# ppwwyyxx/speaker-recognition

Measured on AMD Instinct MI355X. Metric: frames/sec scored (MFCC+GMM), higher is better.
Workload: dtype f32

## Files before the change

speaker-recognition_amd/csrc/abi_options.cpp:

```cpp
#include "abi_internal.hpp"

#include "bw_plan.hpp"
#include "bw_stats.hpp"
#include "calib.hpp"
#include "calib_plan.hpp"
#include "diar.hpp"
#include "diar_plan.hpp"
#include "em.hpp"
#include "featnorm.hpp"
#include "featnorm_plan.hpp"
#include "fork_proxy.hpp"
#include "gmm_full.hpp"
#include "jfa.hpp"
#include "jfa_plan.hpp"
#include "kmeans_init.hpp"
#include "map_batch.hpp"
#include "map_plan.hpp"
#include "mfcc.hpp"
#include "norm_plan.hpp"
#include "plda.hpp"
#include "plda_plan.hpp"
#include "score.hpp"
#include "score_norm.hpp"
#include "silence.hpp"
// ... 18 lines not shown
    const std::string k(key);
    if (k == "score_frames_per_lane") {
        if (value != 0 && value != 1 && value != 2 && value != 4) fail("frames per lane must be 0/1/2/4");
        score_options().frames_per_lane = (int)value;
    } else if (k == "score_model_groups") {
        score_options().model_groups = (int)value;
    } else if (k == "score_packed") {
        score_options().packed = (int)value;
    } else if (k == "score_engine") {
        if (value < 0 || value > 6 || value == 2)
            fail("score_engine must be 0 (auto), 1 (vector ALU), 3 (split-bf16 matrix cores), 4 (split-bf16, shared-sigma form), "
                 "5 (split-fp16 matrix cores) or 6 (split-fp16, shared-sigma form); 2 was the fp32 matrix-core engine, removed in round 5 "
                 "(never selected: 1.45-1.8x slower than split-bf16 at the same accuracy)");
        score_options().engine = (int)value;
    } else if (k == "score_h2s_shape") {
        if (value < 0 || value > 6)
            fail("score_h2s_shape must be 0 (automatic), 1 (4-wave workgroups), 2 (12-wave workgroups), 3 (12 waves, image loop pipelined inside the wave), "
                 "4 (4 waves on one tile, the block's models split between them), 5 (as 3, on the flat image where 3 takes the compact one) "
                 "or 6 (as 3, one quadratic half per block where 3 forms one per two blocks)");
        score_options().h2s_shape = (int)value;
    } else if (k == "flush_list_cap") {
        if (value < 0) fail("flush_list_cap must be >= 0");
        score_options().flush_list_cap = (int)value;
    } else if (k == "score_h2s_pack_tails") {
        if (value != 0 && value != 1) fail("score_h2s_pack_tails must be 0 or 1");
        score_options().h2s_pack_tails = (int)value;
    } else if (k == "score_h2s_force_exc") {
        score_options().h2s_force_exc = value != 0;
    } else if (k == "score_split_shape") {
        if (value != 0 && value != 1 && value != 8 && value != 12 && value != 16)
            fail("score_split_shape must be 0 (automatic), 1 (4-wave workgroups) or 8 / 12 / 16 (waves of the wide, pipelined form)");
        score_options().split_shape = (int)value;
    } else if (k == "score_mfma_ft") {
        if (value < 0 || value > 4) fail("score_mfma_ft must be 0..4");
// ... 92 lines not shown
```

speaker-recognition_amd/csrc/gmm_model.cpp:

```cpp
#include "gmm_model.hpp"
#include "score_shapes.hpp"

#include <atomic>
#include <algorithm>
#include <cmath>
#include <limits>
#include <cstdlib>
#include <cstring>
#include <thread>

namespace sr {
uint64_t next_gmm_uid() {
    static std::atomic<uint64_t> next{1};
    return next.fetch_add(1);
}
}

namespace sr {

namespace {

template <class F>
void host_parallel_for(int n, size_t cost_per_piece, F work) {
    const size_t total = (size_t)n * cost_per_piece;
// ... 746 lines not shown
            }
        }
        amp_t[thr] = amp_l;
        coef_t[thr] = coef_l;
    });
    for (int t = 0; t < MAX_T; t++) {
        pm.amp = std::max(pm.amp, amp_t[t]);
        pm.coef_max = std::max(pm.coef_max, coef_t[t]);
    }
    pm.pad_waste = 1.0 - ((double)K * S) / ((double)pm.n_tiles * MT * n_blocks * SHARED_SB);
    pm.ref = pack_models_split({models[0]}, SPLIT_F16X2);
    return pm;
}

PackedH2Compact pack_h2_compact(const PackedH2Shared &pm, int dim) {
    PackedH2Compact pc;
    if (pm.params.empty() || !h2c_applies(dim, pm.klf)) return pc;
    const int h = h2c_half_steps(dim);
    const H2cMap m = h2c_map(h);
    pc.nk = m.nk;
    pc.nf = m.nf;
    pc.nb = m.nb;
    const int c_slot = 8 * h - 1;
    auto flat_slot = [&](bool linear, int part, int s) {
        if (s < dim) return part == 1 ? s : linear ? 2 * dim + 1 + s : 2 * dim + s;
        if (linear && s == c_slot) return part == 1 ? dim : 3 * dim + 1;
        return -1;
    };
    auto b_desc = [&](bool linear, int part, int s) -> uint16_t {
        if (s < dim) return (uint16_t)(s | ((part == 1 ? 1 : 2) << 8));
        if (linear && s == c_slot && part == 1) return (uint16_t)(3 << 8);
        return 0;
    };
    pc.q_desc.assign((size_t)m.nb * 16, 0);
// ... 98 lines not shown
```

speaker-recognition_amd/csrc/gmm_model.hpp:

```cpp
#pragma once

#include "common.hpp"

#include <memory>
#include <string>
#include <vector>

struct SRModelSet;

namespace sr {
uint64_t next_gmm_uid();
}

struct GMM {
    int nr_mixtures = 0;
    int covariance_type = 1;
    int dim = 0;
    std::vector<double> weights;
    std::vector<double> mean;
    std::vector<double> sigma;
    mutable std::shared_ptr<SRModelSet> single[sr::MAX_DEVICES];
    uint64_t uid = sr::next_gmm_uid();
    uint64_t generation = 0;
    void drop_single() {
// ... 78 lines not shown
    std::vector<uint16_t> params;
    std::vector<SharedBlock> blocks;
    std::vector<float> center, scale;
    std::vector<uint16_t> q_desc, l_desc;
    double amp = 0.0, pad_waste = 0.0, sigma_ratio = 1.0, coef_max = 0.0;
    PackedSplit ref;
};
PackedH2Shared pack_models_h2_shared(const std::vector<const GMM *> &models);
struct PackedH2Compact {
    int nk = 0, nf = 0, nb = 0;
    std::vector<uint16_t> params;
    std::vector<SharedBlock> blocks;
    std::vector<uint16_t> q_desc, l_desc;
};
PackedH2Compact pack_h2_compact(const PackedH2Shared &pm, int dim);
struct WorkItem { int t[4]; };
std::vector<WorkItem> pack_tail_tiles(const std::vector<int> &counts, int frames_per_tile, bool pack_tails);
void mel_sweep_starts(const int *col0, const int *cnt, int n_bands, const int pass_len[4], int *start);
int mel_sweep_extra_cycles(const int *start, const int *cnt, int n_bands, int pass);
bool models_share_sigma_and_weights(const std::vector<const GMM *> &models);
PackedBx3Shared pack_models_bx3_shared(const std::vector<const GMM *> &models);
void split_bf16x3(float v, uint16_t out[3]);
void split_f16x2(float v, uint16_t out[2]);
uint16_t f32_to_f16_rne(float v);
float f16_to_f32(uint16_t h);

}

struct SRModelSet {
    sr::PackedModels host;
// ... 7 lines not shown
    bool bx3_stale = false;
    sr::PackedSplit h2;
    sr::DevBuf<uint16_t> d_h2_params;
    sr::DevBuf<float> d_h2_center, d_h2_scale;
    sr::DevBuf<sr::ChunkDesc> d_h2_chunks;
    sr::PackedBx3Shared shared;
    sr::DevBuf<uint16_t> d_shared_params;
    sr::DevBuf<sr::SharedBlock> d_shared_blocks;
    sr::DevBuf<float> d_shared_center;
    sr::PackedH2Shared h2s;
    sr::DevBuf<uint16_t> d_h2s_params, d_h2s_qdesc, d_h2s_ldesc, d_h2s_ref_params;
    sr::DevBuf<sr::SharedBlock> d_h2s_blocks;
    sr::DevBuf<float> d_h2s_center, d_h2s_scale, d_h2s_ref_center, d_h2s_ref_scale;
    sr::DevBuf<sr::ChunkDesc> d_h2s_ref_chunks;
    sr::DevBuf<int> d_h2s_ref_gcb;
    int h2c_state = 0;
    int h2c_nk = 0;
    sr::DevBuf<uint16_t> d_h2c_params, d_h2c_qdesc, d_h2c_ldesc;
    sr::DevBuf<sr::SharedBlock> d_h2c_blocks;
    struct GroupTable {
        std::vector<int> host;
        sr::DevBuf<int> dev;
    };
    std::vector<std::unique_ptr<GroupTable>> group_tables;
    size_t group_table_next = 0;
    int topc_state = 0;
    sr::DevBuf<float> d_topc_scale;
    sr::DevBuf<float> d_topc_m;
    sr::DevBuf<float> d_topc_c;
    sr::DevBuf<float> d_topc_bg;
    int topc_bg = -1, topc_tp = 0, topc_k = 0;
    sr::DevBuf<int> d_flush_models;
    std::unique_ptr<SRModelSet> hy_good, hy_bad;
    int hy_bad_mixtures = 0;
// ... 3 lines not shown
```

speaker-recognition_amd/csrc/gmm_score_h2_shared.hip:

```cpp
#include "lse.hpp"
#include "score.hpp"
#include "wave_ops.hpp"

#include <algorithm>
#include <cstdint>
#include <type_traits>

namespace sr {

typedef float f32x16 __attribute__((ext_vector_type(16)));
typedef _Float16 f16x8 __attribute__((ext_vector_type(8)));
typedef unsigned u32x4 __attribute__((ext_vector_type(4)));

constexpr int H2S_ROUNDS_PER_LAUNCH = 12;
constexpr float H2S_SUM_LO = 7.8886090522101181e-31f;
constexpr float H2S_SUM_HI = 1.2676506002282294e+30f;
constexpr float H2S_LOG2E = 1.4426950408889634f;

template <int KN, int KM, int COLS>
__device__ __forceinline__ void h2s_chain_regs(f32x16 (&acc)[COLS], const f32x16 (&init)[COLS], const uint4 (&fr)[KM],
                                               const f16x8 (&b)[COLS][KN]) {
#pragma unroll
    for (int ks = 0; ks < KN; ks++)
#pragma unroll
// ... 526 lines not shown
    else if constexpr (NA == 3) { H2P_SLOT_NX(H, R, 3) } \
    else { H2P_SLOT_NX(H, R, 4) }
template <int HEAD, bool READ, int NA, int NX, int W, int O>
__device__ __forceinline__ void h2p_slot(f32x16 &cur, u32x4 &fu, float &s, float &e0, float &e1, float &e2, float &e3, const f16x8 &b, const f32x16 &c,
                                         unsigned at, float p0, float p1, float p2, float p3) {
    static_assert(NA <= 4 && NX <= 4, "at most four exps per slot");
    if constexpr (HEAD == 0) {
        if constexpr (READ) { H2P_SLOT_NA(0, 1) } else { H2P_SLOT_NA(0, 0) }
    } else if constexpr (HEAD == 1) {
        if constexpr (READ) { H2P_SLOT_NA(1, 1) } else { H2P_SLOT_NA(1, 0) }
    } else {
        if constexpr (READ) { H2P_SLOT_NA(2, 1) } else { H2P_SLOT_NA(2, 0) }
    }
}

template <int KQF, int KLF, bool CPT = false, bool PAIR = false>
__global__ __launch_bounds__(12 * 64, 3)
void gmm_score_h2p_kernel(const H2sArgs a) {
    constexpr int SB = SHARED_SB, WAVES = 12, G = 4, NB = 2, DMA_AT = KLF / 2;
    constexpr int KM = KQF > KLF ? KQF : KLF;
    static_assert(KQF <= KLF, "the linear half is never the shorter one");
    static_assert(!CPT || (KQF == H2C_KLF && KLF == H2C_KLF), "the compact order is built for the <8,8> chains");
    static_assert(!CPT || h2c_map_ok(H2C_MAP), "compact order");
    static_assert(!PAIR || (CPT && SB == H2Q_SB && G == H2Q_G), "pairs of blocks: the compact form, blocks of 15, stages of four");
    constexpr int NF = CPT ? H2C_MAP.nf : KM;
    constexpr int NBQ = CPT ? H2C_MAP.nb : KQF, NBL = CPT ? H2C_MAP.nb : KLF;
    constexpr int IMG_U4 = NF * 64;
    constexpr int STAGE_U4 = G * IMG_U4;
    constexpr int N_IMG_T = 1 + SB;
    constexpr int N_IMG = PAIR ? 1 + 2 * SB : 1 + SB;
    constexpr int N_STAGES = N_IMG_T / G;
    static_assert(N_IMG_T % G == 0 && N_STAGES >= 1, "stages tile the images of a mixture tile");
    extern __shared__ uint4 h2s_bq_lds[];
    __shared__ uint4 ring[NB * STAGE_U4];

    const int tid = threadIdx.x;
    const int lane = tid & 63;
    const int wave = __builtin_amdgcn_readfirstlane(tid >> 6);
    const int col = lane & 31;
    const int hh = lane >> 5;

// ... 128 lines not shown
                if (img / G >= n_st) return;
                if constexpr (los) {
                    wait_stages(NB > 2 && S + 2 < n_stage_total ? 1 : 0);
                    barrier();
                    if constexpr (DMA_AT == 0)
                        if (S + NB < n_stage_total) stage_load_next(slot_cur);
                }
                const unsigned next_at = ring_lane + (unsigned)((los ? slot_nxt * STAGE_U4 : slot_cur * STAGE_U4 + (gi + 1) * IMG_U4) * 16);
                f32x16 &cur = img == 0 ? qacc : acc[img & 1];
                const f32x16 &prev = acc[decltype(PSEL)::value];
                constexpr int BW = KQF < 4 ? KQF : 4;
                f16x8 bqt[BW];
                auto bq_load = [&](int ks) { return __builtin_bit_cast(f16x8, h2s_bq_lds[(wave * NBQ + ks) * 64 + lane]); };
                if constexpr (img == 0) {
                    if constexpr (CPT) {
                        h2p_for<0, BW>([&](auto KS) { bqt[decltype(KS)::value] = bq_load(H2C_MAP.b_of[decltype(KS)::value]); });
                    } else {
#pragma unroll
                        for (int ks = 0; ks < BW; ks++) bqt[ks] = bq_load(ks);
                    }
                }
                constexpr bool ONE_ASM = kn >= 5;
                static_assert(!CPT || ONE_ASM, "the compact order is written for the one-statement slots");
                constexpr int sum_model = carry ? prev_model : 0;
                constexpr bool second = PAIR && carry && img != 0 && img - 2 >= SB;
                float &sum_ref = second ? ssum2[second ? img - 2 - SB : 0] : ssum[second ? 0 : sum_model];
                if constexpr (ONE_ASM) {
                    h2p_for<0, kn>([&](auto U) {
                        constexpr int u = decltype(U)::value;
                        if constexpr (los && DMA_AT != 0 && u == DMA_AT)
                            if (S + NB < n_stage_total) stage_load_next(slot_cur);
                        constexpr int fa = CPT ? H2C_MAP.a_of[u] : u, bi = CPT ? H2C_MAP.b_of[u] : u;
                        constexpr bool rd = CPT ? H2C_MAP.a_last[fa] == u : (u < kn_next);
                        constexpr int younger = CPT ? h2c_younger(H2C_MAP, u) : (kn - 1 - u) + (u < kn_next ? u : kn_next);
                        static_assert(younger <= 15, "lgkmcnt is a 4-bit field");
                        constexpr int e0 = carry ? h2p_cum(kn, u - 2) : 0, e1 = carry ? h2p_cum(kn, u - 1) : 0, e2 = carry ? h2p_cum(kn, u) : 0;
                        constexpr int NA = e1 - e0, NX = e2 - e1;
                        const float p0 = prev[e1 < 16 ? e1 : 15], p1 = prev[e1 + 1 < 16 ? e1 + 1 : 15], p2 = prev[e1 + 2 < 16 ? e1 + 2 : 15],
                                    p3 = prev[e1 + 3 < 16 ? e1 + 3 : 15];
                        if constexpr (img == 0)
                        {
                            h2p_slot<u == 0 ? 0 : 2, rd, NA, NX, younger, fa * 1024>(cur, fr[fa], sum_ref, e[0], e[1], e[2], e[3], bqt[u % BW],
                                                                                     qacc, next_at, p0, p1, p2, p3);
                            if constexpr (u + BW < KQF) bqt[u % BW] = bq_load(CPT ? H2C_MAP.b_of[u + BW] : u + BW);
                        }
                        else
                            h2p_slot<u == 0 ? 1 : 2, rd, NA, NX, younger, fa * 1024>(cur, fr[fa], sum_ref, e[0], e[1], e[2], e[3], bl[bi], qacc,
                                                                                     next_at, p0, p1, p2, p3);
                        __builtin_amdgcn_sched_barrier(0);
                    });
                } else {
                    h2p_for<0, kn>([&](auto U) {
                        constexpr int u = decltype(U)::value;
                        if constexpr (los && DMA_AT != 0 && u == DMA_AT)
                            if (S + NB < n_stage_total) stage_load_next(slot_cur);
                        constexpr int younger = (kn - 1 - u) + (u < kn_next ? u : kn_next);
                        u32x4 &fu = fr[u];
                        asm volatile("s_waitcnt lgkmcnt(%1)" : "+v"(fu) : "n"(younger));
                        if constexpr (img == 0)
// ... 281 lines not shown
            const unsigned hot_cols = (unsigned)__builtin_amdgcn_ballot_w64(live && ll < a.band_hi);
            double sum = 0.0;
            for (int j = 0; j < max_pop; j++) {
                const double t = shfl_f64(v, min(excl + j, 31));
                if (j < pop) sum += t;
            }
            if (has && lane < n_ent && si < sb.n_models) {
                double *p = a.partial + (int64_t)ent.x * a.n_models + sb.first_model + si;
                *p = ((hot_cols >> excl) & own_cols) != 0 ? SR_FLUSH_POISON : *p + sum;
            }
            __builtin_amdgcn_sched_barrier(0);
        }
    }
}

template <int KQF, int KLF, int COLS, int WAVES, bool PIN = false, bool MS = false, bool CPT = false, bool PAIR = false>
static int launch_h2s(const H2sLaunch &l) {
    static_assert(!CPT || PIN, "the compact image is the pipelined kernel's");
    static_assert(!PAIR || CPT, "blocks go in pairs on the compact image only");
    constexpr int MQ = CPT ? H2C_KLF : KQF, ML = CPT ? H2C_KLF : KLF;
    constexpr bool BQ_LDS = h2s_bq_in_lds(KQF, KLF, WAVES);
    H2sArgs a;
    a.X = l.X;
    a.tiles = l.tiles;
    a.params = reinterpret_cast<const uint4 *>(l.params);
    a.blocks = l.blocks;
    a.group_block_begin = l.group_block_begin;
    a.center = l.center;
    a.scale = l.scale;
    a.q_desc = l.q_desc;
    a.l_desc = l.l_desc;
    a.ref_ll = l.ref_ll;
    a.partial = l.partial;
    a.frame_ll = l.frame_ll;
// ... 26 lines not shown
    static_assert(!PIN || H2P_ROUND_ITEMS % TILES_WG == 0, "a workgroup's work items never straddle the table's padding");
    int wg_per_launch = WAVES > 4 ? std::max(8, (n_wg + 7) / 8 * 8)
                        : std::max(8, (H2S_ROUNDS_PER_LAUNCH * resident / std::max(1, l.n_groups)) / 8 * 8);
    int n_launches = 0;
    for (int base = 0; base < n_wg; base += wg_per_launch) {
        n_launches++;
        a.tile_base = base * TILES_WG;
        const int n = std::min(wg_per_launch, n_wg - base);
        const int per_xcd = ((l.n_groups + 7) / 8) * n;
        const bool xcd_groups = MS && KLF <= H2M_MAX_KLF && l.n_groups > 1 && n == n_wg && per_xcd <= 2 * (ctx().n_cu / 8);
        dim3 grid(xcd_groups ? (unsigned)(8 * ((l.n_groups + 7) / 8) * n) : (unsigned)((int64_t)l.n_groups * ((n + 7) / 8) * 8));
        a.rows8 = (n + 7) / 8;
        a.n_wg = n;
        a.group_major = xcd_groups ? 2 : l.n_groups > 1;
        constexpr bool M_DIRECT = MS && KLF <= H2M_MAX_KLF;
        constexpr size_t dyn = CPT      ? (size_t)WAVES * H2C_MAP.nb * 64 * sizeof(uint4)
                               : M_DIRECT ? 0
                                          : (BQ_LDS ? (size_t)WAVES * KQF * 64 * sizeof(uint4) : 0) + (MS ? sizeof(uint4) : 0);
        if constexpr (dyn > 0) {
            static bool attr_set[MAX_DEVICES] = {};
            if (!attr_set[ctx().device]) {
                if constexpr (PIN)
                    SR_HIP(hipFuncSetAttribute(reinterpret_cast<const void *>(&gmm_score_h2p_kernel<MQ, ML, CPT, PAIR>),
                                               hipFuncAttributeMaxDynamicSharedMemorySize, (int)dyn));
                else
                    SR_HIP(hipFuncSetAttribute(reinterpret_cast<const void *>(&gmm_score_h2s_kernel<KQF, KLF, COLS, WAVES, MS>),
                                               hipFuncAttributeMaxDynamicSharedMemorySize, (int)dyn));
                attr_set[ctx().device] = true;
            }
        }
        if constexpr (PIN)
            hipLaunchKernelGGL((gmm_score_h2p_kernel<MQ, ML, CPT, PAIR>), grid, dim3(WAVES * 64), dyn, ctx().stream, a);
        else if constexpr (M_DIRECT)
            hipLaunchKernelGGL((gmm_score_h2m_kernel<KQF, KLF>), grid, dim3(WAVES * 64), 0, ctx().stream, a);
        else
            hipLaunchKernelGGL((gmm_score_h2s_kernel<KQF, KLF, COLS, WAVES, MS>), grid, dim3(WAVES * 64), dyn, ctx().stream, a);
    }
    a.tile_base = 0;
    if constexpr (CPT) {
        a.params = reinterpret_cast<const uint4 *>(l.params);
        a.blocks = l.blocks;
        a.q_desc = l.q_desc;
        a.l_desc = l.l_desc;
    }
    if (!a.plan_inline) hipLaunchKernelGGL(h2s_plan_kernel, dim3((unsigned)l.n_blocks), dim3(64), 0, ctx().stream, a);
    const int gy = std::max(1, (2 * ctx().n_cu) / std::max(1, l.n_blocks));
    hipLaunchKernelGGL((gmm_score_h2s_online_kernel<KQF, KLF>), dim3((unsigned)(l.n_blocks * gy)), dim3(256), 0, ctx().stream, a);
    return n_launches;
}

int launch_score_h2_shared(const H2sLaunch &l, int KQF, int KLF) {
#define SR_H2S_CASE(Q, L)                                       \
    if (KQF == Q && KLF == L) {                                 \
        if constexpr (L == H2C_KLF)                             \
            if (l.shape == 2 && l.c_params) return l.pair ? launch_h2s<Q, L, 1, 12, true, false, true, true>(l) : launch_h2s<Q, L, 1, 12, true, false, true>(l); \
        if constexpr (h2p_fits(Q, L))                           \
            if (l.shape == 2) return launch_h2s<Q, L, 1, 12, true>(l); \
        if (l.shape == 3) return launch_h2s<Q, L, 1, 4, false, true>(l); \
        if (l.shape >= 1) return launch_h2s<Q, L, 1, 12>(l);    \
        return launch_h2s<Q, L, 1, 4>(l);                       \
    }
    SR_H2S_CASE(1, 1) SR_H2S_CASE(1, 2) SR_H2S_CASE(2, 2) SR_H2S_CASE(3, 3) SR_H2S_CASE(3, 4) SR_H2S_CASE(4, 4)
    SR_H2S_CASE(4, 5) SR_H2S_CASE(5, 5) SR_H2S_CASE(6, 6) SR_H2S_CASE(6, 7) SR_H2S_CASE(7, 7)
    SR_H2S_CASE(7, 8) SR_H2S_CASE(8, 8) SR_H2S_CASE(9, 9) SR_H2S_CASE(9, 10)
#undef SR_H2S_CASE
    fail("no split-fp16 shared-sigma scoring kernel for %d + %d contraction steps", KQF, KLF);
}

}
```

speaker-recognition_amd/csrc/gmm_score_host.cpp:

```cpp
#include "score.hpp"

#include <algorithm>
#include <cmath>
#include <cstring>

namespace sr {

struct LastKernel {
    char name[256] = "";
};
#define g_last_kernel (per_device<LastKernel>().name)
const char *last_score_kernel() { return g_last_kernel; }

struct PassCounters {
    int *oor_p() { return buf.p; }
    int *flush_count_p() { return buf.p + 1; }
    int *exc_count_p() { return buf.p + 4; }
    int *base() { return buf.p; }
    void begin(size_t n, bool delivering) {
        buf.ensure(n);
        if (!(delivering && clean_p == buf.p && clean_n >= n)) {
            SR_HIP(hipMemsetAsync(buf.p, 0, n * sizeof(int), ctx().stream));
        } else if (score_options().verify_clean_counters) {
            std::vector<int> h(n);
// ... 83 lines not shown
    s.d_h2s_params.upload(h.params.data(), h.params.size());
    s.d_h2s_blocks.upload(h.blocks.data(), h.blocks.size());
    s.d_h2s_center.upload(h.center.data(), h.center.size());
    s.d_h2s_scale.upload(h.scale.data(), h.scale.size());
    s.d_h2s_qdesc.upload(h.q_desc.data(), h.q_desc.size());
    s.d_h2s_ldesc.upload(h.l_desc.data(), h.l_desc.size());
    s.d_h2s_ref_params.upload(h.ref.params.data(), h.ref.params.size());
    s.d_h2s_ref_chunks.upload(h.ref.chunks.data(), h.ref.chunks.size());
    const int gcb[2] = {0, (int)h.ref.chunks.size()};
    s.d_h2s_ref_gcb.upload(gcb, 2);
    s.d_h2s_ref_center.upload(h.ref.center.data(), h.ref.center.size());
    s.d_h2s_ref_scale.upload(h.ref.scale.data(), h.ref.scale.size());
    sync_stream();
}

static bool ensure_h2c_layout(SRModelSet &s) {
    if (s.h2c_state != 0) return s.h2c_state > 0;
    const PackedH2Shared &h = s.h2s;
    if (!h2c_built(s.host.dim, h.klf)) {
        s.h2c_state = -1;
        return false;
    }
    const PackedH2Compact c = pack_h2_compact(h, s.host.dim);
    const size_t pad_u16 = (size_t)c.nf * 64 * 8;
    s.d_h2c_params.ensure(c.params.size() + pad_u16);
    s.d_h2c_params.upload(c.params.data(), c.params.size());
    SR_HIP(hipMemsetAsync(s.d_h2c_params.p + c.params.size(), 0, pad_u16 * sizeof(uint16_t), ctx().stream));
    s.d_h2c_blocks.upload(c.blocks.data(), c.blocks.size());
    s.d_h2c_qdesc.upload(c.q_desc.data(), c.q_desc.size());
    s.d_h2c_ldesc.upload(c.l_desc.data(), c.l_desc.size());
    sync_stream();
    s.h2c_nk = c.nk;
    s.h2c_state = 1;
    return true;
}

static void ensure_h2_layout(SRModelSet &s) {
    if (s.d_h2_params.p) return;
    s.d_h2_params.upload(s.h2.params.data(), s.h2.params.size());
    s.d_h2_chunks.upload(s.h2.chunks.data(), s.h2.chunks.size());
    s.d_h2_center.upload(s.h2.center.data(), s.h2.center.size());
    s.d_h2_scale.upload(s.h2.scale.data(), s.h2.scale.size());
    sync_stream();
}

void ensure_bx3_layout(SRModelSet &s) {
    if (s.d_bx3_params.p && !s.bx3_stale) return;
    s.bx3_stale = false;
// ... 81 lines not shown
    a.blocks = set.d_h2s_blocks.p;
    a.group_block_begin = c.d_gcb;
    a.center = set.d_h2s_center.p;
    a.scale = set.d_h2s_scale.p;
    a.q_desc = set.d_h2s_qdesc.p;
    a.l_desc = set.d_h2s_ldesc.p;
    a.ref_ll = w.ref_ll.p;
    a.oor_flag = w.counters.oor_p();
    a.exc_list = w.exc_list.p;
    a.exc_count = w.counters.exc_count_p();
    a.n_blocks = n_blocks;
    a.n_mix_tiles = h.n_tiles;
    a.log2_k = (float)std::log2((double)h.n_tiles * MT);
    a.force_exc = opt.h2s_force_exc;
    a.shape = h2s_shape;
    bool compact = false;
    if (h2s_shape == 2) {
        ensure_work_table(tt, opt.h2s_pack_tails != 0);
        a.tiles = tt.d_tiles_work.p;
        a.n_work = tt.n_work;
        compact = opt.h2s_shape != 5 && ensure_h2c_layout(set);
        if (compact) {
            a.pair = opt.h2s_shape != 6;
            a.c_params = set.d_h2c_params.p;
            a.c_blocks = set.d_h2c_blocks.p;
            a.c_q_desc = set.d_h2c_qdesc.p;
            a.c_l_desc = set.d_h2c_ldesc.p;
        }
    }
    snprintf(g_last_kernel, sizeof(LastKernel::name),
             "%s<%d,%d,%s>%s (shared sigma: quadratic half once per %d models; split-fp16 MFMA, "
             "3 products as one contraction; reference-offset log-sum-exp)", h2s_shape == 2 ? "gmm_score_h2p_kernel" : (h2s_shape == 3 && h2s_msplit_direct(h.klf)) ? "gmm_score_h2m_kernel" : "gmm_score_h2s_kernel",
             compact ? set.h2c_nk : h.kqf, compact ? set.h2c_nk : h.klf,
             h2s_shape == 2 ? "waves=12, pipelined in the wave" : h2s_shape == 1 ? "waves=12" : h2s_shape == 3 ? "waves=4 on one tile, models split" : "waves=4",
             compact ? "/compact" : "", a.pair ? 2 * SHARED_SB : SHARED_SB);
    ScopedKernelTimer t(T_SCORE);
    const int n_launches = launch_score_h2_shared(a, h.kqf, h.klf);
    const size_t len = strlen(g_last_kernel);
    snprintf(g_last_kernel + len, sizeof(LastKernel::name) - len, " [%d launches per pass]", n_launches);
}

static void launch_shared_bf16(SRModelSet &set, const PassArgs &c) {
    ensure_shared_layout(set);
    SharedLaunch a = common_args<SharedLaunch>(c);
    a.params = set.d_shared_params.p;
    a.blocks = set.d_shared_blocks.p;
    a.group_block_begin = c.d_gcb;
    a.center = set.d_shared_center.p;
    a.n_mix_tiles = set.shared.n_tiles;
    snprintf(g_last_kernel, sizeof(LastKernel::name),
// ... 405 lines not shown
```

speaker-recognition_amd/csrc/score.hpp:

```cpp
#pragma once

#include "batch.hpp"
#include "gmm_model.hpp"
#include "score_plan.hpp"

namespace sr {

constexpr int SCORE_NO_FLUSH = 0x400;
constexpr int SCORE_HOST_DELIVER = 0x800;
constexpr size_t HOST_DELIVER_MAX_BYTES = (size_t)64 << 10;
constexpr size_t HOST_DELIVER_MAX_UTTS = 256;
inline bool host_deliverable(size_t n_utt, size_t n_models) {
    return n_utt > 0 && n_utt <= HOST_DELIVER_MAX_UTTS && n_utt * n_models * sizeof(double) + n_utt * sizeof(int) <= HOST_DELIVER_MAX_BYTES;
}
struct DeliverHeader {
    int oor, n_flush;
    unsigned seq;
    int pad;
};

struct ScoreArgs {
    const float *X;
    const TileDesc *tiles;
    const float4 *params;
// ... 64 lines not shown
    float *frame_ll;
    int *oor_flag;
    int n_work = 0;
    int *exc_list;
    int *exc_count;
    int n_blocks;
    int64_t n_frames;
    int dim, n_models, n_mix_tiles, clamp, n_groups, n_tiles;
    float log2_k;
    int force_exc;
    int shape = 0;
    const uint16_t *c_params = nullptr;
    const SharedBlock *c_blocks = nullptr;
    const uint16_t *c_q_desc = nullptr, *c_l_desc = nullptr;
    bool pair = false;
    float band_hi = -__builtin_inff();
};
int launch_score_h2_shared(const H2sLaunch &a, int KQF, int KLF);
void launch_score_split(const MfmaLaunch &a, int scheme, int KS, int FT);
bool launch_score_splitp(const MfmaLaunch &a, int scheme, int KS, int waves, int chunks_per_model);
const char *last_score_kernel();

struct ScoreResult {
    const double *d_sums = nullptr;
    const int *d_argmax = nullptr;
    const float *d_frame_ll = nullptr;
    const int *d_oor = nullptr;
    const int *d_flush_count = nullptr;
    const int2 *d_flush_list = nullptr;
    int flush_cap = 0;
// ... 71 lines not shown
```

speaker-recognition_amd/csrc/score_plan.cpp:

```cpp
#include "score_plan.hpp"

#include <algorithm>
#include <cmath>

namespace sr {

ScoreOptions &score_options() {
    static ScoreOptions o;
    return o;
}

static int auto_frames_per_lane(int64_t n_rows, int n_utt, int dp) {
    const int fmax = dp <= 40 ? 4 : dp <= 64 ? 2 : 1;
    if (n_utt == 0) return 1;
    const double mean_len = (double)n_rows / n_utt;
    for (int f = fmax; f > 1; f >>= 1) {
        const double tile = 256.0 * f;
        const double tiles = std::ceil(mean_len / tile);
        if (mean_len / (tiles * tile) >= 0.80) return f;
    }
    return 1;
}

static Engine precise_engine(const SRModelSet &set) {
// ... 38 lines not shown
    ScorePlan p;
    p.engine = pick_engine(set, opt.engine, (flags & SCORE_PRECISE) != 0);
    const PackedSplit &split = p.engine == Engine::SPLIT_F16 ? set.h2 : set.bx3;
    int F = opt.frames_per_lane ? opt.frames_per_lane : auto_frames_per_lane(n_rows, n_utt, DP);
    if (DP > 40 && F > 2) F = 2;
    if (DP > 64) F = 1;
    if (!opt.frames_per_lane)
        while (F > 1 && ((n_rows + 256 * F - 1) / (256 * F)) * (int64_t)std::max(1, S) < 2 * (int64_t)n_cu) F >>= 1;
    p.F = F;
    if (p.split()) p.FT = opt.mfma_ft ? std::min(opt.mfma_ft, split_max_ft(split.ks)) : 1;
    const int64_t n32 = (n_rows + 31) / 32 + n_utt;
    if (p.engine == Engine::SHARED_F16) {
        const bool wide = n32 >= 64 + n_utt;
        const int64_t ms_wgs = n32 * (int64_t)set.h2s.blocks.size();
        const bool tiny = ms_wgs <= (int64_t)n_cu * (h2s_msplit_direct(set.h2s.klf) ? 2 : 1);
        p.h2s_shape = (opt.h2s_shape == 5 || opt.h2s_shape == 6) ? H2S_PIPELINED_SHAPE : opt.h2s_shape ? opt.h2s_shape - 1 : (tiny ? H2S_MSPLIT_SHAPE : wide ? H2S_PIPELINED_SHAPE : 0);
        if (p.h2s_shape == H2S_PIPELINED_SHAPE && !h2p_fits(set.h2s.kqf, set.h2s.klf)) p.h2s_shape = H2S_WIDE_SHAPE;
    }
    if (p.engine == Engine::SPLIT_F16 && p.FT == 1 && opt.split_shape != 1) {
        const std::vector<int> &mcb = split.model_chunk_begin;
        p.split_cpm = S > 0 ? mcb[1] - mcb[0] : 0;
        for (int s = 1; s < S; s++)
            if (mcb[s + 1] - mcb[s] != p.split_cpm) p.split_cpm = 0;
        if (p.split_cpm > 0) {
            const int w = splitp_waves_f16x2(split.ks, opt.split_shape ? opt.split_shape : 8);
            if (w > 0 && (opt.split_shape || (split.ks >= 5 && (int64_t)S * p.split_cpm >= 32 &&
                                              (n32 / w) * (int64_t)std::min(S, 16) >= (int64_t)6 * n_cu * splitp_resident_per_cu(w))))
                p.splitp_w = w;
        }
    }
    const bool mat = p.engine != Engine::VECTOR;
// ... 169 lines not shown
```

speaker-recognition_amd/csrc/score_shapes.hpp:

```cpp
#pragma once

#include <initializer_list>

#if defined(__HIPCC__)
#define SR_HD __host__ __device__
#else
#define SR_HD
#endif

namespace sr {

SR_HD constexpr int h2s_waves_per_eu(int kqf, int klf, int cols, int waves, bool ms = false) {
    (void)kqf; (void)klf; (void)cols; (void)ms;
    return waves > 4 ? waves / 4 : 2;
}
constexpr int H2M_MAX_KLF = 9;
SR_HD constexpr bool h2p_fits(int kqf, int klf) { return klf >= 2 && kqf <= klf && (2 * 4 * klf + 12 * kqf) * 1024 <= 160 * 1024; }

constexpr int H2C_MAX_STEPS = 16;
struct H2cMap {
    int h = 0, nk = 0, nf = 0, nb = 0;
    int a_of[H2C_MAX_STEPS] = {}, b_of[H2C_MAX_STEPS] = {};
    int a_last[H2C_MAX_STEPS] = {}, b_last[H2C_MAX_STEPS] = {};
    int a_half[H2C_MAX_STEPS][2] = {}, b_half[H2C_MAX_STEPS][2] = {};
// ... 21 lines not shown
        m.b_half[2 * np][0] = h - 1;            m.b_half[2 * np][1] = 16 + h - 1;
        m.b_half[2 * np + 1][0] = 16 + h - 1;   m.b_half[2 * np + 1][1] = -1;
    }
    int k = 0;
    for (int i = 0; i < np; i++, k++) { m.a_of[k] = i;      m.b_of[k] = i; }
    for (int i = 0; i < np; i++, k++) { m.a_of[k] = i;      m.b_of[k] = np + i; }
    if (odd) { m.a_of[k] = np; m.b_of[k] = 2 * np; k++; }
    for (int i = 0; i < np; i++, k++) { m.a_of[k] = nh + i; m.b_of[k] = np + i; }
    if (odd) { m.a_of[k] = nh + np; m.b_of[k] = 2 * np + 1; k++; }
    for (int s = 0; s < m.nk; s++) {
        m.a_last[m.a_of[s]] = s;
        m.b_last[m.b_of[s]] = s;
    }
    return m;
}
SR_HD constexpr int h2c_younger(const H2cMap &m, int u) {
    const int lu = m.a_last[m.a_of[u]];
    int n = 0;
    for (int f = 0; f < m.nf; f++) n += (m.a_last[f] > lu) + (m.a_last[f] < u);
    return n;
}
SR_HD constexpr bool h2c_map_ok(const H2cMap &m) {
    if (m.nk > H2C_MAX_STEPS || m.nf > m.nk || m.nb > m.nk || m.nk != h2c_steps(m.h)) return false;
    for (int f = 0; f < m.nf; f++) {
        bool used = false;
        for (int s = 0; s < m.nk; s++) used = used || m.a_of[s] == f;
        if (!used || (f > 0 && m.a_last[f] <= m.a_last[f - 1])) return false;
    }
    for (int r = 0; r < m.nb; r++) {
        bool used = false;
        for (int s = 0; s < m.nk; s++) used = used || m.b_of[s] == r;
        if (!used) return false;
    }
    for (int s = 0; s < m.nk; s++)
        if (m.a_of[s] < 0 || m.a_of[s] >= m.nf || m.b_of[s] < 0 || m.b_of[s] >= m.nb || h2c_younger(m, s) > 15) return false;
    return true;
}
constexpr int H2C_KLF = 8, H2C_H = 5;
constexpr H2cMap H2C_MAP = h2c_map(H2C_H);
static_assert(h2c_map_ok(h2c_map(H2C_H)) && h2c_map(H2C_H).nk == H2C_KLF && h2c_map(H2C_H).nf == 6 && h2c_map(H2C_H).nb == 6, "the compact order of the <8,8> chains");
static_assert(h2c_map_ok(h2c_map(4)) && h2c_map_ok(h2c_map(3)) && h2c_map_ok(h2c_map(6)) && h2c_map_ok(h2c_map(1)), "even and odd part lengths");
SR_HD constexpr bool h2c_built(int dim, int klf) { return klf == H2C_KLF && h2c_applies(dim, klf) && h2c_half_steps(dim) == H2C_H; }
SR_HD constexpr int h2c_lds_bytes(int h) { return (2 * 4 * h2c_map(h).nf + 12 * h2c_map(h).nb) * 1024; }
static_assert(h2c_lds_bytes(H2C_H) <= 160 * 1024 && (4 * h2c_map(H2C_H).nf) % 12 == 0, "the compact ring fits a CU; a stage is a whole number of pieces per wave");

constexpr int H2Q_SB = 15, H2Q_G = 4;
SR_HD constexpr bool h2q_pairs(int sb, int m1, int m2) { return m2 > 0 && m1 == sb; }
SR_HD constexpr int h2q_stages(int g, int m1, int m2) { return (1 + m1 + m2 + g - 1) / g; }
SR_HD constexpr int h2q_images(int sb, int g, int m1, int m2) {
    return h2q_stages(g, m1, m2) * g < 1 + 2 * sb ? h2q_stages(g, m1, m2) * g : 1 + 2 * sb;
}
SR_HD constexpr int h2q_last_image(int sb, int g, int m1, int m2) { return h2q_images(sb, g, m1, m2) - 1; }
SR_HD constexpr int h2q_last_parity(int sb, int g, int m1, int m2) { return h2q_last_image(sb, g, m1, m2) & 1; }
SR_HD constexpr int h2q_last_model(int sb, int g, int m1, int m2) { return h2q_last_image(sb, g, m1, m2) - 1; }
SR_HD constexpr int h2q_stage_block(int sb, int g, int s) { return s * g < 1 + sb ? 0 : 1; }
SR_HD constexpr int h2q_stage_image(int sb, int g, int s) { return s * g < 1 + sb ? s * g : s * g - sb; }
static_assert((1 + H2Q_SB) % H2Q_G == 0 && h2q_stages(H2Q_G, H2Q_SB, H2Q_SB) == 8 && h2q_images(H2Q_SB, H2Q_G, H2Q_SB, H2Q_SB) == 31 &&
              h2q_last_parity(H2Q_SB, H2Q_G, H2Q_SB, H2Q_SB) == 0 && h2q_last_parity(H2Q_SB, H2Q_G, H2Q_SB, 6) == 1 &&
              h2q_stage_image(H2Q_SB, H2Q_G, 4) == 1 && h2q_stage_image(H2Q_SB, H2Q_G, 7) == 13, "a full pair: 31 images, the last an even one");
// ... 41 lines not shown
```

Baseline: 39.32 million.

## Pack odd-length compact image into five fragments by joining the two odd tails

Adds a joined compact map that stores the two odd half-steps of the <8,8> chains in one shared fragment, so the compact image holds five fragments per model where it held six. It becomes the default compact layout, with the six-fragment map kept as shape 7 for comparison. The aim is to cut the per-image bytes streamed into LDS and the ring size (112 KiB instead of 120 KiB). The cost is a different fragment reuse order inside the pipelined loop, which changes its wait counts and its scheduling.

```diff
diff --git a/speaker-recognition_amd/csrc/abi_options.cpp b/speaker-recognition_amd/csrc/abi_options.cpp
--- a/speaker-recognition_amd/csrc/abi_options.cpp
+++ b/speaker-recognition_amd/csrc/abi_options.cpp
@@ -56,10 +56,11 @@
                  "(never selected: 1.45-1.8x slower than split-bf16 at the same accuracy)");
         score_options().engine = (int)value;
     } else if (k == "score_h2s_shape") {
-        if (value < 0 || value > 6)
+        if (value < 0 || value > 7)
             fail("score_h2s_shape must be 0 (automatic), 1 (4-wave workgroups), 2 (12-wave workgroups), 3 (12 waves, image loop pipelined inside the wave), "
-                 "4 (4 waves on one tile, the block's models split between them), 5 (as 3, on the flat image where 3 takes the compact one) "
-                 "or 6 (as 3, one quadratic half per block where 3 forms one per two blocks)");
+                 "4 (4 waves on one tile, the block's models split between them), 5 (as 3, on the flat image where 3 takes the compact one), "
+                 "6 (as 3, one quadratic half per block where 3 forms one per two blocks) or 7 (as 3, on the compact image of six stored "
+                 "fragments where 3 takes the one of five)");
         score_options().h2s_shape = (int)value;
     } else if (k == "flush_list_cap") {
         if (value < 0) fail("flush_list_cap must be >= 0");
diff --git a/speaker-recognition_amd/csrc/gmm_model.cpp b/speaker-recognition_amd/csrc/gmm_model.cpp
--- a/speaker-recognition_amd/csrc/gmm_model.cpp
+++ b/speaker-recognition_amd/csrc/gmm_model.cpp
@@ -784,10 +784,14 @@
 }
 
 PackedH2Compact pack_h2_compact(const PackedH2Shared &pm, int dim) {
+    return pack_h2_compact(pm, dim, h2c_map(h2c_half_steps(dim)));
+}
+
+PackedH2Compact pack_h2_compact(const PackedH2Shared &pm, int dim, const H2cMap &m) {
     PackedH2Compact pc;
     if (pm.params.empty() || !h2c_applies(dim, pm.klf)) return pc;
     const int h = h2c_half_steps(dim);
-    const H2cMap m = h2c_map(h);
+    if (m.h != h || !h2c_map_ok(m)) fail("pack_h2_compact: the map is not one of %d half-steps per part", h);
     pc.nk = m.nk;
     pc.nf = m.nf;
     pc.nb = m.nb;
diff --git a/speaker-recognition_amd/csrc/gmm_model.hpp b/speaker-recognition_amd/csrc/gmm_model.hpp
--- a/speaker-recognition_amd/csrc/gmm_model.hpp
+++ b/speaker-recognition_amd/csrc/gmm_model.hpp
@@ -116,6 +116,8 @@
     std::vector<uint16_t> q_desc, l_desc;
 };
 PackedH2Compact pack_h2_compact(const PackedH2Shared &pm, int dim);
+struct H2cMap;
+PackedH2Compact pack_h2_compact(const PackedH2Shared &pm, int dim, const H2cMap &m);
 struct WorkItem { int t[4]; };
 std::vector<WorkItem> pack_tail_tiles(const std::vector<int> &counts, int frames_per_tile, bool pack_tails);
 void mel_sweep_starts(const int *col0, const int *cnt, int n_bands, const int pass_len[4], int *start);
@@ -153,10 +155,13 @@
     sr::DevBuf<float> d_h2s_center, d_h2s_scale, d_h2s_ref_center, d_h2s_ref_scale;
     sr::DevBuf<sr::ChunkDesc> d_h2s_ref_chunks;
     sr::DevBuf<int> d_h2s_ref_gcb;
-    int h2c_state = 0;
-    int h2c_nk = 0;
-    sr::DevBuf<uint16_t> d_h2c_params, d_h2c_qdesc, d_h2c_ldesc;
-    sr::DevBuf<sr::SharedBlock> d_h2c_blocks;
+    struct H2cDevice {
+        int state = 0;
+        sr::DevBuf<uint16_t> params, qdesc, ldesc;
+        sr::DevBuf<sr::SharedBlock> blocks;
+    };
+    H2cDevice h2c;
+    H2cDevice h2c_six;
     struct GroupTable {
         std::vector<int> host;
         sr::DevBuf<int> dev;
diff --git a/speaker-recognition_amd/csrc/gmm_score_h2_shared.hip b/speaker-recognition_amd/csrc/gmm_score_h2_shared.hip
--- a/speaker-recognition_amd/csrc/gmm_score_h2_shared.hip
+++ b/speaker-recognition_amd/csrc/gmm_score_h2_shared.hip
@@ -564,17 +564,17 @@
     }
 }
 
-template <int KQF, int KLF, bool CPT = false, bool PAIR = false>
+template <int KQF, int KLF, bool CPT = false, bool PAIR = false, bool SIX = false>
 __global__ __launch_bounds__(12 * 64, 3)
 void gmm_score_h2p_kernel(const H2sArgs a) {
     constexpr int SB = SHARED_SB, WAVES = 12, G = 4, NB = 2, DMA_AT = KLF / 2;
     constexpr int KM = KQF > KLF ? KQF : KLF;
     static_assert(KQF <= KLF, "the linear half is never the shorter one");
     static_assert(!CPT || (KQF == H2C_KLF && KLF == H2C_KLF), "the compact order is built for the <8,8> chains");
-    static_assert(!CPT || h2c_map_ok(H2C_MAP), "compact order");
+    static_assert(!CPT || h2c_map_ok(H2C_MAP_OF<SIX>), "compact order");
     static_assert(!PAIR || (CPT && SB == H2Q_SB && G == H2Q_G), "pairs of blocks: the compact form, blocks of 15, stages of four");
-    constexpr int NF = CPT ? H2C_MAP.nf : KM;
-    constexpr int NBQ = CPT ? H2C_MAP.nb : KQF, NBL = CPT ? H2C_MAP.nb : KLF;
+    constexpr int NF = CPT ? H2C_MAP_OF<SIX>.nf : KM;
+    constexpr int NBQ = CPT ? H2C_MAP_OF<SIX>.nb : KQF, NBL = CPT ? H2C_MAP_OF<SIX>.nb : KLF;
     constexpr int IMG_U4 = NF * 64;
     constexpr int STAGE_U4 = G * IMG_U4;
     constexpr int N_IMG_T = 1 + SB;
@@ -733,7 +733,7 @@
                 auto bq_load = [&](int ks) { return __builtin_bit_cast(f16x8, h2s_bq_lds[(wave * NBQ + ks) * 64 + lane]); };
                 if constexpr (img == 0) {
                     if constexpr (CPT) {
-                        h2p_for<0, BW>([&](auto KS) { bqt[decltype(KS)::value] = bq_load(H2C_MAP.b_of[decltype(KS)::value]); });
+                        h2p_for<0, BW>([&](auto KS) { bqt[decltype(KS)::value] = bq_load(H2C_MAP_OF<SIX>.b_of[decltype(KS)::value]); });
                     } else {
 #pragma unroll
                         for (int ks = 0; ks < BW; ks++) bqt[ks] = bq_load(ks);
@@ -749,9 +749,9 @@
                         constexpr int u = decltype(U)::value;
                         if constexpr (los && DMA_AT != 0 && u == DMA_AT)
                             if (S + NB < n_stage_total) stage_load_next(slot_cur);
-                        constexpr int fa = CPT ? H2C_MAP.a_of[u] : u, bi = CPT ? H2C_MAP.b_of[u] : u;
-                        constexpr bool rd = CPT ? H2C_MAP.a_last[fa] == u : (u < kn_next);
-                        constexpr int younger = CPT ? h2c_younger(H2C_MAP, u) : (kn - 1 - u) + (u < kn_next ? u : kn_next);
+                        constexpr int fa = CPT ? H2C_MAP_OF<SIX>.a_of[u] : u, bi = CPT ? H2C_MAP_OF<SIX>.b_of[u] : u;
+                        constexpr bool rd = CPT ? H2C_MAP_OF<SIX>.a_last[fa] == u : (u < kn_next);
+                        constexpr int younger = CPT ? h2c_younger(H2C_MAP_OF<SIX>, u) : (kn - 1 - u) + (u < kn_next ? u : kn_next);
                         static_assert(younger <= 15, "lgkmcnt is a 4-bit field");
                         constexpr int e0 = carry ? h2p_cum(kn, u - 2) : 0, e1 = carry ? h2p_cum(kn, u - 1) : 0, e2 = carry ? h2p_cum(kn, u) : 0;
                         constexpr int NA = e1 - e0, NX = e2 - e1;
@@ -761,7 +761,7 @@
                         {
                             h2p_slot<u == 0 ? 0 : 2, rd, NA, NX, younger, fa * 1024>(cur, fr[fa], sum_ref, e[0], e[1], e[2], e[3], bqt[u % BW],
                                                                                      qacc, next_at, p0, p1, p2, p3);
-                            if constexpr (u + BW < KQF) bqt[u % BW] = bq_load(CPT ? H2C_MAP.b_of[u + BW] : u + BW);
+                            if constexpr (u + BW < KQF) bqt[u % BW] = bq_load(CPT ? H2C_MAP_OF<SIX>.b_of[u + BW] : u + BW);
                         }
                         else
                             h2p_slot<u == 0 ? 1 : 2, rd, NA, NX, younger, fa * 1024>(cur, fr[fa], sum_ref, e[0], e[1], e[2], e[3], bl[bi], qacc,
@@ -1073,10 +1073,11 @@
     }
 }
 
-template <int KQF, int KLF, int COLS, int WAVES, bool PIN = false, bool MS = false, bool CPT = false, bool PAIR = false>
+template <int KQF, int KLF, int COLS, int WAVES, bool PIN = false, bool MS = false, bool CPT = false, bool PAIR = false, bool SIX = false>
 static int launch_h2s(const H2sLaunch &l) {
     static_assert(!CPT || PIN, "the compact image is the pipelined kernel's");
     static_assert(!PAIR || CPT, "blocks go in pairs on the compact image only");
+    static_assert(!SIX || PAIR, "the six-fragment image: the parent's paired kernel, kept for A/B");
     constexpr int MQ = CPT ? H2C_KLF : KQF, ML = CPT ? H2C_KLF : KLF;
     constexpr bool BQ_LDS = h2s_bq_in_lds(KQF, KLF, WAVES);
     H2sArgs a;
@@ -1133,14 +1134,14 @@
         a.n_wg = n;
         a.group_major = xcd_groups ? 2 : l.n_groups > 1;
         constexpr bool M_DIRECT = MS && KLF <= H2M_MAX_KLF;
-        constexpr size_t dyn = CPT      ? (size_t)WAVES * H2C_MAP.nb * 64 * sizeof(uint4)
+        constexpr size_t dyn = CPT      ? (size_t)WAVES * H2C_MAP_OF<SIX>.nb * 64 * sizeof(uint4)
                                : M_DIRECT ? 0
                                           : (BQ_LDS ? (size_t)WAVES * KQF * 64 * sizeof(uint4) : 0) + (MS ? sizeof(uint4) : 0);
         if constexpr (dyn > 0) {
             static bool attr_set[MAX_DEVICES] = {};
             if (!attr_set[ctx().device]) {
                 if constexpr (PIN)
-                    SR_HIP(hipFuncSetAttribute(reinterpret_cast<const void *>(&gmm_score_h2p_kernel<MQ, ML, CPT, PAIR>),
+                    SR_HIP(hipFuncSetAttribute(reinterpret_cast<const void *>(&gmm_score_h2p_kernel<MQ, ML, CPT, PAIR, SIX>),
                                                hipFuncAttributeMaxDynamicSharedMemorySize, (int)dyn));
                 else
                     SR_HIP(hipFuncSetAttribute(reinterpret_cast<const void *>(&gmm_score_h2s_kernel<KQF, KLF, COLS, WAVES, MS>),
@@ -1149,7 +1150,7 @@
             }
         }
         if constexpr (PIN)
-            hipLaunchKernelGGL((gmm_score_h2p_kernel<MQ, ML, CPT, PAIR>), grid, dim3(WAVES * 64), dyn, ctx().stream, a);
+            hipLaunchKernelGGL((gmm_score_h2p_kernel<MQ, ML, CPT, PAIR, SIX>), grid, dim3(WAVES * 64), dyn, ctx().stream, a);
         else if constexpr (M_DIRECT)
             hipLaunchKernelGGL((gmm_score_h2m_kernel<KQF, KLF>), grid, dim3(WAVES * 64), 0, ctx().stream, a);
         else
@@ -1172,7 +1173,13 @@
 #define SR_H2S_CASE(Q, L)                                       \
     if (KQF == Q && KLF == L) {                                 \
         if constexpr (L == H2C_KLF)                             \
-            if (l.shape == 2 && l.c_params) return l.pair ? launch_h2s<Q, L, 1, 12, true, false, true, true>(l) : launch_h2s<Q, L, 1, 12, true, false, true>(l); \
+            if (l.shape == 2 && l.c_params) {                   \
+                if (l.six) {                                    \
+                    if (!l.pair) fail("the six-fragment compact image is kept for the paired form only"); \
+                    return launch_h2s<Q, L, 1, 12, true, false, true, true, true>(l); \
+                }                                               \
+                return l.pair ? launch_h2s<Q, L, 1, 12, true, false, true, true>(l) : launch_h2s<Q, L, 1, 12, true, false, true>(l); \
+            }                                                   \
         if constexpr (h2p_fits(Q, L))                           \
             if (l.shape == 2) return launch_h2s<Q, L, 1, 12, true>(l); \
         if (l.shape == 3) return launch_h2s<Q, L, 1, 4, false, true>(l); \
diff --git a/speaker-recognition_amd/csrc/gmm_score_host.cpp b/speaker-recognition_amd/csrc/gmm_score_host.cpp
--- a/speaker-recognition_amd/csrc/gmm_score_host.cpp
+++ b/speaker-recognition_amd/csrc/gmm_score_host.cpp
@@ -121,24 +121,24 @@
     sync_stream();
 }
 
-static bool ensure_h2c_layout(SRModelSet &s) {
-    if (s.h2c_state != 0) return s.h2c_state > 0;
+static bool ensure_h2c_layout(SRModelSet &s, bool six) {
+    SRModelSet::H2cDevice &d = six ? s.h2c_six : s.h2c;
+    if (d.state != 0) return d.state > 0;
     const PackedH2Shared &h = s.h2s;
     if (!h2c_built(s.host.dim, h.klf)) {
-        s.h2c_state = -1;
+        d.state = -1;
         return false;
     }
-    const PackedH2Compact c = pack_h2_compact(h, s.host.dim);
+    const PackedH2Compact c = pack_h2_compact(h, s.host.dim, six ? H2C_MAP_SIX : H2C_MAP);
     const size_t pad_u16 = (size_t)c.nf * 64 * 8;
-    s.d_h2c_params.ensure(c.params.size() + pad_u16);
-    s.d_h2c_params.upload(c.params.data(), c.params.size());
-    SR_HIP(hipMemsetAsync(s.d_h2c_params.p + c.params.size(), 0, pad_u16 * sizeof(uint16_t), ctx().stream));
-    s.d_h2c_blocks.upload(c.blocks.data(), c.blocks.size());
-    s.d_h2c_qdesc.upload(c.q_desc.data(), c.q_desc.size());
-    s.d_h2c_ldesc.upload(c.l_desc.data(), c.l_desc.size());
-    sync_stream();
-    s.h2c_nk = c.nk;
-    s.h2c_state = 1;
+    d.params.ensure(c.params.size() + pad_u16);
+    d.params.upload(c.params.data(), c.params.size());
+    SR_HIP(hipMemsetAsync(d.params.p + c.params.size(), 0, pad_u16 * sizeof(uint16_t), ctx().stream));
+    d.blocks.upload(c.blocks.data(), c.blocks.size());
+    d.qdesc.upload(c.q_desc.data(), c.q_desc.size());
+    d.ldesc.upload(c.l_desc.data(), c.l_desc.size());
+    sync_stream();
+    d.state = 1;
     return true;
 }
 
@@ -250,26 +250,29 @@
     a.log2_k = (float)std::log2((double)h.n_tiles * MT);
     a.force_exc = opt.h2s_force_exc;
     a.shape = h2s_shape;
-    bool compact = false;
+    bool compact = false, six = false;
     if (h2s_shape == 2) {
         ensure_work_table(tt, opt.h2s_pack_tails != 0);
         a.tiles = tt.d_tiles_work.p;
         a.n_work = tt.n_work;
-        compact = opt.h2s_shape != 5 && ensure_h2c_layout(set);
+        six = opt.h2s_shape == 7;
+        compact = opt.h2s_shape != 5 && ensure_h2c_layout(set, six);
         if (compact) {
+            const SRModelSet::H2cDevice &d = six ? set.h2c_six : set.h2c;
             a.pair = opt.h2s_shape != 6;
-            a.c_params = set.d_h2c_params.p;
-            a.c_blocks = set.d_h2c_blocks.p;
-            a.c_q_desc = set.d_h2c_qdesc.p;
-            a.c_l_desc = set.d_h2c_ldesc.p;
+            a.six = six;
+            a.c_params = d.params.p;
+            a.c_blocks = d.blocks.p;
+            a.c_q_desc = d.qdesc.p;
+            a.c_l_desc = d.ldesc.p;
         }
     }
     snprintf(g_last_kernel, sizeof(LastKernel::name),
              "%s<%d,%d,%s>%s (shared sigma: quadratic half once per %d models; split-fp16 MFMA, "
              "3 products as one contraction; reference-offset log-sum-exp)", h2s_shape == 2 ? "gmm_score_h2p_kernel" : (h2s_shape == 3 && h2s_msplit_direct(h.klf)) ? "gmm_score_h2m_kernel" : "gmm_score_h2s_kernel",
-             compact ? set.h2c_nk : h.kqf, compact ? set.h2c_nk : h.klf,
+             compact ? H2C_KLF : h.kqf, compact ? H2C_KLF : h.klf,
              h2s_shape == 2 ? "waves=12, pipelined in the wave" : h2s_shape == 1 ? "waves=12" : h2s_shape == 3 ? "waves=4 on one tile, models split" : "waves=4",
-             compact ? "/compact" : "", a.pair ? 2 * SHARED_SB : SHARED_SB);
+             compact ? (six ? "/compact, six fragments" : "/compact") : "", a.pair ? 2 * SHARED_SB : SHARED_SB);
     ScopedKernelTimer t(T_SCORE);
     const int n_launches = launch_score_h2_shared(a, h.kqf, h.klf);
     const size_t len = strlen(g_last_kernel);
diff --git a/speaker-recognition_amd/csrc/score.hpp b/speaker-recognition_amd/csrc/score.hpp
--- a/speaker-recognition_amd/csrc/score.hpp
+++ b/speaker-recognition_amd/csrc/score.hpp
@@ -102,6 +102,7 @@
     const SharedBlock *c_blocks = nullptr;
     const uint16_t *c_q_desc = nullptr, *c_l_desc = nullptr;
     bool pair = false;
+    bool six = false;
     float band_hi = -__builtin_inff();
 };
 int launch_score_h2_shared(const H2sLaunch &a, int KQF, int KLF);
diff --git a/speaker-recognition_amd/csrc/score_plan.cpp b/speaker-recognition_amd/csrc/score_plan.cpp
--- a/speaker-recognition_amd/csrc/score_plan.cpp
+++ b/speaker-recognition_amd/csrc/score_plan.cpp
@@ -76,7 +76,7 @@
         const bool wide = n32 >= 64 + n_utt;
         const int64_t ms_wgs = n32 * (int64_t)set.h2s.blocks.size();
         const bool tiny = ms_wgs <= (int64_t)n_cu * (h2s_msplit_direct(set.h2s.klf) ? 2 : 1);
-        p.h2s_shape = (opt.h2s_shape == 5 || opt.h2s_shape == 6) ? H2S_PIPELINED_SHAPE : opt.h2s_shape ? opt.h2s_shape - 1 : (tiny ? H2S_MSPLIT_SHAPE : wide ? H2S_PIPELINED_SHAPE : 0);
+        p.h2s_shape = (opt.h2s_shape >= 5 && opt.h2s_shape <= 7) ? H2S_PIPELINED_SHAPE : opt.h2s_shape ? opt.h2s_shape - 1 : (tiny ? H2S_MSPLIT_SHAPE : wide ? H2S_PIPELINED_SHAPE : 0);
         if (p.h2s_shape == H2S_PIPELINED_SHAPE && !h2p_fits(set.h2s.kqf, set.h2s.klf)) p.h2s_shape = H2S_WIDE_SHAPE;
     }
     if (p.engine == Engine::SPLIT_F16 && p.FT == 1 && opt.split_shape != 1) {
diff --git a/speaker-recognition_amd/csrc/score_shapes.hpp b/speaker-recognition_amd/csrc/score_shapes.hpp
--- a/speaker-recognition_amd/csrc/score_shapes.hpp
+++ b/speaker-recognition_amd/csrc/score_shapes.hpp
@@ -59,6 +59,35 @@
     }
     return m;
 }
+SR_HD constexpr H2cMap h2c_map_joined(int h) {
+    if ((h & 1) == 0) return h2c_map(h);
+    H2cMap m;
+    m.h = h;
+    m.nk = h2c_steps(h);
+    const int np = h / 2;
+    m.nf = h;
+    m.nb = h + 1;
+    for (int i = 0; i < np; i++) {
+        m.a_half[i][0] = 2 * i;                 m.a_half[i][1] = 2 * i + 1;
+        m.a_half[np + 1 + i][0] = 16 + 2 * i;   m.a_half[np + 1 + i][1] = 16 + 2 * i + 1;
+        m.b_half[i][0] = 2 * i;                 m.b_half[i][1] = 2 * i + 1;
+        m.b_half[np + i][0] = 16 + 2 * i;       m.b_half[np + i][1] = 16 + 2 * i + 1;
+    }
+    m.a_half[np][0] = h - 1;                    m.a_half[np][1] = 16 + h - 1;
+    m.b_half[2 * np][0] = h - 1;                m.b_half[2 * np][1] = 16 + h - 1;
+    m.b_half[2 * np + 1][0] = 16 + h - 1;       m.b_half[2 * np + 1][1] = -1;
+    int k = 0;
+    for (int i = 0; i < np; i++, k++) { m.a_of[k] = i;          m.b_of[k] = i; }
+    for (int i = 0; i < np; i++, k++) { m.a_of[k] = i;          m.b_of[k] = np + i; }
+    m.a_of[k] = np; m.b_of[k] = 2 * np; k++;
+    m.a_of[k] = np; m.b_of[k] = 2 * np + 1; k++;
+    for (int i = 0; i < np; i++, k++) { m.a_of[k] = np + 1 + i; m.b_of[k] = np + i; }
+    for (int s = 0; s < m.nk; s++) {
+        m.a_last[m.a_of[s]] = s;
+        m.b_last[m.b_of[s]] = s;
+    }
+    return m;
+}
 SR_HD constexpr int h2c_younger(const H2cMap &m, int u) {
     const int lu = m.a_last[m.a_of[u]];
     int n = 0;
@@ -82,12 +111,18 @@
     return true;
 }
 constexpr int H2C_KLF = 8, H2C_H = 5;
-constexpr H2cMap H2C_MAP = h2c_map(H2C_H);
-static_assert(h2c_map_ok(h2c_map(H2C_H)) && h2c_map(H2C_H).nk == H2C_KLF && h2c_map(H2C_H).nf == 6 && h2c_map(H2C_H).nb == 6, "the compact order of the <8,8> chains");
+constexpr H2cMap H2C_MAP = h2c_map_joined(H2C_H);
+constexpr H2cMap H2C_MAP_SIX = h2c_map(H2C_H);
+template <bool SIX> constexpr H2cMap H2C_MAP_OF = SIX ? H2C_MAP_SIX : H2C_MAP;
+static_assert(h2c_map_ok(H2C_MAP) && H2C_MAP.nk == H2C_KLF && H2C_MAP.nf == 5 && H2C_MAP.nb == 6, "the joined order of the <8,8> chains");
+static_assert(h2c_map_ok(H2C_MAP_SIX) && H2C_MAP_SIX.nk == H2C_KLF && H2C_MAP_SIX.nf == 6 && H2C_MAP_SIX.nb == 6, "the six-fragment order of the <8,8> chains");
 static_assert(h2c_map_ok(h2c_map(4)) && h2c_map_ok(h2c_map(3)) && h2c_map_ok(h2c_map(6)) && h2c_map_ok(h2c_map(1)), "even and odd part lengths");
+static_assert(h2c_map_ok(h2c_map_joined(1)) && h2c_map_ok(h2c_map_joined(2)) && h2c_map_ok(h2c_map_joined(3)) && h2c_map_ok(h2c_map_joined(4)) &&
+              h2c_map_ok(h2c_map_joined(5)) && h2c_map_ok(h2c_map_joined(6)) && h2c_map_ok(h2c_map_joined(7)) && h2c_map_ok(h2c_map_joined(8)) &&
+              h2c_map_ok(h2c_map_joined(9)) && h2c_map_ok(h2c_map_joined(10)), "the joined map at every part length");
 SR_HD constexpr bool h2c_built(int dim, int klf) { return klf == H2C_KLF && h2c_applies(dim, klf) && h2c_half_steps(dim) == H2C_H; }
-SR_HD constexpr int h2c_lds_bytes(int h) { return (2 * 4 * h2c_map(h).nf + 12 * h2c_map(h).nb) * 1024; }
-static_assert(h2c_lds_bytes(H2C_H) <= 160 * 1024 && (4 * h2c_map(H2C_H).nf) % 12 == 0, "the compact ring fits a CU; a stage is a whole number of pieces per wave");
+SR_HD constexpr int h2c_lds_bytes(const H2cMap &m) { return (2 * 4 * m.nf + 12 * m.nb) * 1024; }
+static_assert(h2c_lds_bytes(H2C_MAP) == 112 * 1024 && h2c_lds_bytes(H2C_MAP_SIX) == 120 * 1024, "40 + 72 and 48 + 72 KiB of a CU's 160");
 
 constexpr int H2Q_SB = 15, H2Q_G = 4;
 SR_HD constexpr bool h2q_pairs(int sb, int m1, int m2) { return m2 > 0 && m1 == sb; }
```

After: 39.54 million, median of 6. No clear change (+0.5%).
